# atunnd/Hair-centric-Image-Retrieval

Hardware: AMD Instinct MI355X
Metric: query-images/sec (embed+top-10) ViT-B/16 vs 1M gallery, 1/2/4/8 GPU (higher is better)
Workload: dtype f16; 1 GPU; ViT-B/16 (HSimCLR ViTWrapper, random init) embed + top-10 over 1000000 x 768 f32 gallery row-sharded over 1 GPU(s); query_batch_per_gpu=880, global_query_batch=880, gallery_rows=1000000, gallery_dtype=f32, topk=10, sim_mode=filtered, residual_stream=f16, steps_in_flight=2, parallelism=gallery-shard1+query-dp1

## Files before the change

### hair-centric-image-retrieval_amd/csrc/gemm.hip

```cpp
#include "sim_core.h"
#include "act.h"
#include "gemm_plan.h"
#include <stdlib.h>

namespace {

using GemmCfg = SimCfg<_Float16, 2, 2, 2>;

constexpr int EPI_RESID_F16_STATS = 7;
constexpr int EPI_LN_BIAS_F16 = 8;
constexpr int EPI_LN_BIAS_GELU_F16 = 9;
constexpr int EPI_BIAS_F16_DUAL_GELU = 10;

struct GemmArgs {
  const _Float16* a;
  const _Float16* w;
  const float* bias;
  const float* scale;
  void* out;
  int64_t m, lda, ldw, ldo;
  int n, k;
  const float* ln_stats;
  const float* ln_c1;
  float* stats_part;
  const void* resid;
  void* out2;
  int64_t stats_ld = 0;
};

__device__ __forceinline__ int xcd_remap(int bid, int nwg) {
  const int q = nwg >> 3, r = nwg & 7, xcd = bid & 7, j = bid >> 3;
  return (xcd < r ? xcd * (q + 1) : r * (q + 1) + (xcd - r) * q) + j;
}

template <int EPI, int NTILES>
// ... 70 lines not shown
  gemm_epilogue_t<EPI, 2>(g, acc, m0, n0 + wave_n * 64, wave_m, lane);
}
__device__ __forceinline__ void launder(f32x4& v) { asm volatile("" : "+v"(v)); }

struct WaveAcc {
  f32x4 a[8][4];
  __device__ __forceinline__ void zero() {
#pragma unroll
    for (int x = 0; x < 8; ++x)
#pragma unroll
      for (int y = 0; y < 4; ++y)
#pragma unroll
        for (int i = 0; i < 4; ++i) a[x][y][i] = 0.f;
  }
};

__device__ __forceinline__ float sum8_dpp(float v) {
  v += __builtin_bit_cast(float, __builtin_amdgcn_update_dpp(0, __builtin_bit_cast(int, v), 0xB1, 0xF, 0xF, true));
  v += __builtin_bit_cast(float, __builtin_amdgcn_update_dpp(0, __builtin_bit_cast(int, v), 0x4E, 0xF, 0xF, true));
  v += __builtin_bit_cast(float, __builtin_amdgcn_update_dpp(0, __builtin_bit_cast(int, v), 0x141, 0xF, 0xF, true));
  return v;
}


template <int EPI, bool FULL, int NTW, int MTT, int MTH>
__device__ __forceinline__ void gemm_epilogue_lds_impl(const GemmArgs& g, const f32x4 (&acc)[NTW][MTT], int mt0,
                                                       char* region, int64_t m0w, int nbase, int lane) {
  constexpr bool kLn = (EPI == EPI_LN_BIAS_F16 || EPI == EPI_LN_BIAS_GELU_F16);
  constexpr bool kGelu = (EPI == HCIR_EPI_BIAS_GELU_F16 || EPI == EPI_LN_BIAS_GELU_F16);
  constexpr bool kResidH = (EPI == HCIR_EPI_BIAS_RESID_F16 || EPI == EPI_RESID_F16_STATS);
  constexpr bool kDual = (EPI == EPI_BIAS_F16_DUAL_GELU);
  constexpr bool kF16 = (EPI == HCIR_EPI_BIAS_F16 || kGelu || kLn ||
                         EPI == HCIR_EPI_AFFINE_RELU_F16 || kResidH || kDual);
  constexpr bool kAffine = (EPI == HCIR_EPI_AFFINE_RELU_F16 || EPI == HCIR_EPI_AFFINE_F32);
  constexpr int FPP = kF16 ? 64 : 32;
  constexpr int NPASS = NTW * 16 / FPP;
  constexpr int NIT = MTH * 2;
  constexpr int UB = (NIT % 4 == 0) ? 4 : 3;
  static_assert(NIT % UB == 0 && (NTW * 16) % FPP == 0, "geometry");
  const int rrow = lane >> 3, rchunk = lane & 7;

  constexpr bool kScaleA = kF16 && (EPI == HCIR_EPI_AFFINE_RELU_F16 || kResidH);
  f32x4 biasA[kF16 ? NTW : 1], scaleA[kScaleA ? NTW : 1];
  bool has_scale = false;
  if constexpr (kF16) {
    has_scale = kScaleA && (EPI == HCIR_EPI_AFFINE_RELU_F16 || g.scale != nullptr);
#pragma unroll
    for (int t = 0; t < NTW; ++t) {
      const int n = nbase + 16 * t + 4 * (lane >> 4);
      biasA[t] = (f32x4){0.f, 0.f, 0.f, 0.f};
      if (g.bias) biasA[t] = *reinterpret_cast<const f32x4*>(g.bias + n);
      if constexpr (kScaleA) {
        scaleA[t] = (f32x4){1.f, 1.f, 1.f, 1.f};
        if (has_scale) scaleA[t] = *reinterpret_cast<const f32x4*>(g.scale + n);
      }
    }
// ... 6 lines not shown
#pragma unroll
    for (int j = 0; j < NB; ++j) {
      const int n = nbase + pass * FPP + rchunk * (kF16 ? 8 : 4) + 4 * j;
      bias[pass][j] = (f32x4){0.f, 0.f, 0.f, 0.f};
      scale[pass][j] = (f32x4){1.f, 1.f, 1.f, 1.f};
      if (g.bias) bias[pass][j] = *reinterpret_cast<const f32x4*>(g.bias + n);
      if (kAffine || (EPI == HCIR_EPI_BIAS_RESID_F32 && g.scale))
        scale[pass][j] = *reinterpret_cast<const f32x4*>(g.scale + n);
    }
  }
  float ln_rs[MTH], ln_mean[MTH];
  f32x4 c1a[NTW];
  if constexpr (kLn) {
#pragma unroll
    for (int mt = 0; mt < MTH; ++mt) {
      int64_t mm = m0w + 16 * mt + (lane & 15);
      mm = mm < g.m ? mm : g.m - 1;
      ln_mean[mt] = g.ln_stats[2 * mm];
      ln_rs[mt] = g.ln_stats[2 * mm + 1];
    }
#pragma unroll
    for (int t = 0; t < NTW; ++t) c1a[t] = *reinterpret_cast<const f32x4*>(g.ln_c1 + nbase + 16 * t + 4 * (lane >> 4));
  }
  asm volatile("s_waitcnt vmcnt(0)" ::: "memory");
  if constexpr (kLn) {
#pragma unroll
    for (int mt = 0; mt < MTH; ++mt) asm volatile("" : "+v"(ln_rs[mt]));
#pragma unroll
    for (int mt = 0; mt < MTH; ++mt) asm volatile("" : "+v"(ln_mean[mt]));
#pragma unroll
    for (int t = 0; t < NTW; ++t) launder(c1a[t]);
  }
  if constexpr (kF16) {
#pragma unroll
    for (int t = 0; t < NTW; ++t) {
      launder(biasA[t]);
      if constexpr (kScaleA) launder(scaleA[t]);
    }
  } else {
#pragma unroll
    for (int pass = 0; pass < NPASS; ++pass)
#pragma unroll
      for (int j = 0; j < NB; ++j) {
        launder(bias[pass][j]);
        launder(scale[pass][j]);
      }
  }

  constexpr int NITER = kDual ? 2 * NPASS : NPASS;
#pragma unroll
  for (int iter = 0; iter < NITER; ++iter) {
    const int pass = kDual ? iter >> 1 : iter;
    const bool second = kDual && (iter & 1);
    const int r16 = lane & 15, q16 = lane >> 4;
#pragma unroll
    for (int mt = 0; mt < MTH; ++mt) {
      const int row = mt * 16 + r16;
      if constexpr (kF16) {
#pragma unroll
        for (int q = 0; q < 4; ++q) {
          const int nt = 4 * pass + q;
          f16x4 o;
          float xs[4];
#pragma unroll
          for (int e = 0; e < 4; ++e) {
            float x = acc[nt][mt0 + mt][e];
            const float bb = biasA[nt][e];
            if constexpr (kLn) {
              x = __builtin_fmaf(ln_rs[mt], __builtin_fmaf(-ln_mean[mt], c1a[nt][e], x), bb);
            } else if constexpr (EPI == HCIR_EPI_AFFINE_RELU_F16) {
              x = fmaxf(__builtin_fmaf(x, scaleA[nt][e], bb), 0.f);
            } else if constexpr (kResidH) {
              x = scaleA[nt][e] * (x + bb);
            } else {
              x += bb;
            }
            xs[e] = x;
          }
          if (kGelu || second) {
#pragma unroll
            for (int e = 0; e < 4; e += 2) {
              const gelu_f32x2 y = gelu_erf2((gelu_f32x2){xs[e], xs[e + 1]});
              xs[e] = y[0];
              xs[e + 1] = y[1];
            }
          }
#pragma unroll
          for (int e = 0; e < 4; ++e) o[e] = (_Float16)xs[e];
          const int chunk = 2 * q + (q16 >> 1);
          *reinterpret_cast<f16x4*>(region + row * 128 + ((chunk ^ (row & 7)) << 4) + 8 * (q16 & 1)) = o;
        }
      } else {
#pragma unroll
        for (int q = 0; q < 2; ++q) {
          const int nt = 2 * pass + q;
          const int chunk = 4 * q + q16;
// ... 5 lines not shown
      const int n = nbase + pass * 64 + rchunk * 8;
#pragma unroll
      for (int it0 = 0; it0 < NIT; it0 += UB) {
        f16x8 oldh[UB];
        if constexpr (kResidH) {
#pragma unroll
          for (int u = 0; u < UB; ++u) {
            const int64_t mm = m0w + (it0 + u) * 8 + rrow;
#pragma unroll
            for (int e = 0; e < 8; ++e) oldh[u][e] = (_Float16)0.f;
            if (FULL || mm < g.m)
              oldh[u] = *reinterpret_cast<const f16x8*>(static_cast<const _Float16*>(g.resid) + mm * g.ldo + n);
          }
        }
#pragma unroll
        for (int u = 0; u < UB; ++u) {
          const int row = (it0 + u) * 8 + rrow;
          const f16x8 v = *reinterpret_cast<const f16x8*>(region + row * 128 + ((rchunk ^ (row & 7)) << 4));
          f16x8 o;
          if constexpr (kResidH)
            o = v + oldh[u];
          else
            o = v;
          const int64_t m = m0w + row;
          if (FULL || m < g.m)
            __builtin_nontemporal_store(
                o, reinterpret_cast<f16x8*>(static_cast<_Float16*>(second ? g.out2 : g.out) + m * g.ldo + n));
          if constexpr (EPI == EPI_RESID_F16_STATS) {
            float xv[8], s1 = 0.f;
#pragma unroll
            for (int e = 0; e < 8; ++e) {
              xv[e] = (float)o[e];
              s1 += xv[e];
            }
            const float mean_s = sum8_dpp(s1) * (1.0f / 64.0f);
            float m2 = 0.f;
#pragma unroll
            for (int e = 0; e < 8; ++e) {
              const float dv = xv[e] - mean_s;
              m2 = __builtin_fmaf(dv, dv, m2);
            }
            m2 = sum8_dpp(m2);
            if (rchunk == 0 && (FULL || m < g.m)) {
              const int64_t slice = (nbase >> 6) + pass;
              *reinterpret_cast<f32x2*>(g.stats_part + (slice * (g.stats_ld ? g.stats_ld : g.m) + m) * 2) = (f32x2){mean_s, m2};
            }
          }
        }
      }
    } else {
      const int n = nbase + pass * 32 + rchunk * 4;
      const f32x4 b = bias[pass][0], sc = scale[pass][0];
#pragma unroll
      for (int it0 = 0; it0 < NIT; it0 += UB) {
        f32x4 oldv[UB];
#pragma unroll
        for (int u = 0; u < UB; ++u) {
          const int64_t mm = m0w + (it0 + u) * 8 + rrow;
          oldv[u] = (f32x4){0.f, 0.f, 0.f, 0.f};
          if constexpr (EPI == HCIR_EPI_BIAS_RESID_F32) {
            if (FULL || mm < g.m)
              oldv[u] = *reinterpret_cast<const f32x4*>(static_cast<const float*>(g.resid) + mm * g.ldo + n);
          }
        }
#pragma unroll
        for (int u = 0; u < UB; ++u) {
          const int row = (it0 + u) * 8 + rrow;
          const int64_t mm = m0w + row;
          f32x4 v = *reinterpret_cast<const f32x4*>(region + row * 128 + ((rchunk ^ (row & 7)) << 4));
          if constexpr (EPI == HCIR_EPI_AFFINE_F32) {
#pragma unroll
            for (int e = 0; e < 4; ++e) v[e] = __builtin_fmaf(v[e], sc[e], b[e]);
          } else if constexpr (EPI == HCIR_EPI_BIAS_RESID_F32) {
#pragma unroll
            for (int e = 0; e < 4; ++e) v[e] = __builtin_fmaf(sc[e], v[e] + b[e], oldv[u][e]);
          } else {
#pragma unroll
            for (int e = 0; e < 4; ++e) v[e] += b[e];
          }
          if (FULL || mm < g.m) *reinterpret_cast<f32x4*>(static_cast<float*>(g.out) + mm * g.ldo + n) = v;
        }
      }
    }
  }
}

template <int EPI, int NTW, int MTT, int MTH>
__device__ __forceinline__ void gemm_epilogue_lds(const GemmArgs& g, const f32x4 (&acc)[NTW][MTT], int mt0,
                                                  char* region, int64_t m0w, int nbase, int lane) {
  asm volatile("" : "+v"(lane));
  if (m0w + 16 * MTH <= g.m)
    gemm_epilogue_lds_impl<EPI, true, NTW, MTT, MTH>(g, acc, mt0, region, m0w, nbase, lane);
  else
    gemm_epilogue_lds_impl<EPI, false, NTW, MTT, MTH>(g, acc, mt0, region, m0w, nbase, lane);
}

template <int EPI, bool GLDS>
__global__ __launch_bounds__(256, 2) void gemm_f16_kernel(GemmArgs g, int tiles_n, int tiles_m) {
  using Cfg = GemmCfg;
  __shared__ __attribute__((aligned(16))) char lds[Cfg::LDS_BYTES];
  const int tid = threadIdx.x, lane = tid & 63, wave = tid >> 6;
  const int wave_n = wave >> 1, wave_m = wave & 1;
  const int t = xcd_remap(blockIdx.x, tiles_n * tiles_m);
  const int tn = t % tiles_n, tm = t / tiles_n;
  const int n0 = tn * 128;
  const int64_t m0 = (int64_t)tm * 128;
  const int nkc = (g.k + 63) / 64;

  f32x16 acc[2][2];
#pragma unroll
  for (int a = 0; a < 2; ++a)
// ... 447 lines not shown
#pragma unroll
        for (int e = 0; e < 4; ++e) v[e] = acc[nt][mt][4 * grp + e] + b[e] + p.pos_mult * ps[e];
        if constexpr (sizeof(TokT) == 4) {
          *reinterpret_cast<f32x4*>(orow + n) = v;
        } else {
          f16x4 o;
#pragma unroll
          for (int e = 0; e < 4; ++e) o[e] = (_Float16)v[e];
          *reinterpret_cast<f16x4*>(orow + n) = o;
        }
      }
    }
  }
}

template <typename TokT>
__global__ void cls_row_kernel(const float* __restrict__ cls, const float* __restrict__ pos,
                               float pos_mult, int64_t b, int t, int d, TokT* __restrict__ tok) {
  const int64_t i = (int64_t)blockIdx.x * blockDim.x + threadIdx.x;
  if (i >= b * d) return;
  const int64_t bi = i / d;
  const int n = (int)(i % d);
  tok[bi * t * (int64_t)d + n] = (TokT)(cls[n] + pos_mult * pos[n]);
}

__global__ void ln_stats_finalize_kernel(const float* __restrict__ part, int parts, int64_t m, float slice_n,
                                         float eps, float* __restrict__ stats) {
  const int64_t row = (int64_t)blockIdx.x * blockDim.x + threadIdx.x;
  if (row >= m) return;
  float ms = 0.f;
  for (int p = 0; p < parts; ++p) ms += part[((int64_t)p * m + row) * 2];
  const float mean = ms / (float)parts;
  float m2 = 0.f;
  for (int p = 0; p < parts; ++p) {
    const f32x2 v = *reinterpret_cast<const f32x2*>(part + ((int64_t)p * m + row) * 2);
    const float dm = v[0] - mean;
    m2 += v[1] + slice_n * dm * dm;
  }
  const float var = m2 / (slice_n * (float)parts);
  *reinterpret_cast<f32x2*>(stats + 2 * row) = (f32x2){mean, 1.0f / sqrtf(var + eps)};
}

template <int EPI>
void launch_gemm_mid(const GemmArgs& g, hipStream_t st) {
  const int tn = g.n / GMid::TN, tm = (int)hcir_cdiv(g.m, GMid::TM);
  const int grid = tn * tm < 512 ? tn * tm : 512;
// ... 124 lines not shown

int hcir_gemm_f16_fused(const void* a, int64_t lda, const void* w, int64_t ldw, const float* bias,
                        const float* scale, int64_t m, int32_t n, int32_t k, int epilogue, void* out,
                        int64_t ldo, const float* ln_stats, const float* ln_c1, float* stats_part,
                        void* stream) {
  HCIR_ENTER();
  if (!a || !w || !out || m <= 0 || n <= 0 || k <= 0) return HCIR_ERR_INVALID;
  if ((k & 7) || (n & 7) || lda < k || ldw < k || (lda & 7) || (ldw & 7) || ldo < n || (ldo & 7))
    return HCIR_ERR_INVALID;
  const bool ln = ln_stats || ln_c1;
  if (ln && (!ln_stats || !ln_c1 || !bias)) return HCIR_ERR_INVALID;
  if (ln && stats_part) return HCIR_ERR_INVALID;
  if (!ln && !stats_part) return HCIR_ERR_INVALID;
  if (ln && epilogue != HCIR_EPI_BIAS_F16 && epilogue != HCIR_EPI_BIAS_GELU_F16) return HCIR_ERR_UNSUPPORTED;
  if (stats_part && epilogue != HCIR_EPI_BIAS_RESID_F16) return HCIR_ERR_UNSUPPORTED;
  if (!gemm_takes_big(m, n, k)) return HCIR_ERR_UNSUPPORTED;
  GemmArgs g{static_cast<const _Float16*>(a), static_cast<const _Float16*>(w), bias, scale, out, m,
             lda, ldw, ldo, n, k, ln_stats, ln_c1, stats_part, out, nullptr};
  hipStream_t st = static_cast<hipStream_t>(stream);
  const GemmPlan p = gemm_plan(m, n, k, false);
  if (stats_part) launch_gemm_big<EPI_RESID_F16_STATS>(g, p, st);
  else if (epilogue == HCIR_EPI_BIAS_F16) launch_gemm_big<EPI_LN_BIAS_F16>(g, p, st);
  else launch_gemm_big<EPI_LN_BIAS_GELU_F16>(g, p, st);
  HCIR_LAUNCH_CHECK();
  return HCIR_OK;
}

int hcir_ln_stats_finalize(const float* stats_part, int32_t slices, int64_t m, int32_t n_features, float eps,
                           float* ln_stats, void* stream) {
  HCIR_ENTER();
  if (!stats_part || !ln_stats || slices <= 0 || m <= 0 || n_features <= 0) return HCIR_ERR_INVALID;
  if ((int64_t)slices * 64 != n_features) return HCIR_ERR_INVALID;
  hipLaunchKernelGGL(ln_stats_finalize_kernel, dim3((unsigned)hcir_cdiv(m, 256)), dim3(256), 0,
                     static_cast<hipStream_t>(stream), stats_part, slices, m, 64.0f, eps, ln_stats);
  HCIR_LAUNCH_CHECK();
  return HCIR_OK;
}

int hcir_patch_embed(const float* img, int64_t b, int32_t c, int32_t h, int32_t w_px, int32_t p,
                     const void* w_f16, int64_t ldw, const float* bias, const float* cls,
                     const float* pos, float pos_mult, int32_t d, void* tok, int tok_dtype,
                     void* stream) {
  HCIR_ENTER();
  if (!img || !w_f16 || !bias || !cls || !pos || !tok || b <= 0) return HCIR_ERR_INVALID;
  if (p <= 0 || p > 32 || c <= 0 || h % p || w_px % p || (d & 7)) return HCIR_ERR_INVALID;
  const int kreal = c * p * p;
// ... 6 lines not shown
  if (tok_dtype != HCIR_F32 && tok_dtype != HCIR_F16) return HCIR_ERR_UNSUPPORTED;
  const dim3 cgrid((unsigned)hcir_cdiv(b * d, 256));
  if (tok_dtype == HCIR_F32) {
    if (p == 16)
      hipLaunchKernelGGL((patch_embed_kernel<float, true>), dim3(tiles_n * tiles_m), dim3(256), 0, st, a, tiles_n, tiles_m);
    else
      hipLaunchKernelGGL((patch_embed_kernel<float, false>), dim3(tiles_n * tiles_m), dim3(256), 0, st, a, tiles_n, tiles_m);
    HCIR_LAUNCH_CHECK();
    hipLaunchKernelGGL(cls_row_kernel<float>, cgrid, dim3(256), 0, st, cls, pos, pos_mult, b, np + 1, d,
                       static_cast<float*>(tok));
  } else {
    if (p == 16)
      hipLaunchKernelGGL((patch_embed_kernel<_Float16, true>), dim3(tiles_n * tiles_m), dim3(256), 0, st, a, tiles_n, tiles_m);
    else
      hipLaunchKernelGGL((patch_embed_kernel<_Float16, false>), dim3(tiles_n * tiles_m), dim3(256), 0, st, a, tiles_n, tiles_m);
    HCIR_LAUNCH_CHECK();
    hipLaunchKernelGGL(cls_row_kernel<_Float16>, cgrid, dim3(256), 0, st, cls, pos, pos_mult, b, np + 1, d,
                       static_cast<_Float16*>(tok));
  }
  HCIR_LAUNCH_CHECK();
  return HCIR_OK;
}

}
```

### hair-centric-image-retrieval_amd/hcir/_lib.py

```python
from __future__ import annotations

import ctypes
import os
import subprocess

import torch

_PKG_DIR = os.path.dirname(os.path.dirname(os.path.abspath(__file__)))
CSRC_DIR = os.path.join(_PKG_DIR, "csrc")
LIB_PATH = os.environ.get("HCIR_LIB_PATH") or os.path.join(CSRC_DIR, "libhcir.so")

F32, F16, BF16 = 0, 1, 2
EPI_BIAS_F16, EPI_BIAS_GELU_F16, EPI_BIAS_RESID_F32, EPI_BIAS_F32, EPI_AFFINE_RELU_F16, EPI_AFFINE_F32, \
    EPI_BIAS_RESID_F16 = range(7)
GEMM_ROUTE_SMALL, GEMM_ROUTE_MID, GEMM_ROUTE_BIG, GEMM_ROUTE_SPLIT = range(4)
GEMM_ROUTE_EPI_DUAL = 10

_lib = None

c_i32, c_i64, c_f32, c_vp, c_sz, c_int = (
    ctypes.c_int32, ctypes.c_int64, ctypes.c_float, ctypes.c_void_p, ctypes.c_size_t, ctypes.c_int)
c_f64 = ctypes.c_double

SIGNATURES = {
    "hcir_version": (c_int, []),
    "hcir_status_string": (ctypes.c_char_p, [c_int]),
    "hcir_build_id": (ctypes.c_char_p, []),
    "hcir_row_invnorm": (c_int, [c_vp, c_i64, c_i32, c_i64, c_int, c_f32, c_vp, c_vp]),
    "hcir_l2_normalize": (c_int, [c_vp, c_i64, c_i32, c_f32, c_vp, c_vp, c_vp]),
    "hcir_sim_topk_workspace_bytes": (c_sz, [c_i64, c_i64, c_i32, c_i32, c_int]),
    "hcir_sim_topk": (c_int, [c_vp, c_i64, c_vp, c_i64, c_i32, c_i32, c_int, c_vp, c_vp, c_i64,
                              c_vp, c_vp, c_vp, c_sz, c_vp]),
    "hcir_topk_refine_f32": (c_int, [c_vp, c_i64, c_vp, c_i64, c_i32, c_vp, c_vp, c_i32, c_i32, c_i64, c_vp, c_vp,
                                     c_vp, c_vp, c_vp, c_vp, c_vp, c_vp]),
    "hcir_topk_merge": (c_int, [c_vp, c_vp, c_i32, c_i64, c_i32, c_i32, c_vp, c_vp, c_vp]),
    "hcir_ntxent_workspace_bytes": (c_sz, [c_i64, c_i32, c_int]),
    "hcir_ntxent_fwd": (c_int, [c_vp, c_vp, c_i64, c_i32, c_int, c_f32, c_vp, c_vp, c_vp, c_sz, c_vp]),
    "hcir_ntxent_bwd_workspace_bytes": (c_sz, [c_i64, c_i32, c_int]),
    "hcir_ntxent_bwd": (c_int, [c_vp, c_vp, c_i64, c_i32, c_int, c_f32, c_vp, c_f32, c_vp, c_vp, c_vp, c_sz, c_vp]),
    "hcir_layernorm_f16": (c_int, [c_vp, c_int, c_i64, c_i32, c_i64, c_vp, c_vp, c_f32, c_vp, c_i64, c_vp]),
    "hcir_gemm_f16": (c_int, [c_vp, c_i64, c_vp, c_i64, c_vp, c_vp, c_i64, c_i32, c_i32, c_int,
                              c_vp, c_i64, c_vp]),
    "hcir_gemm_f16_resid": (c_int, [c_vp, c_i64, c_vp, c_i64, c_vp, c_vp, c_i64, c_i32, c_i32, c_int, c_vp,
                                    c_vp, c_i64, c_vp]),
    "hcir_gemm_f16_gelu_dual": (c_int, [c_vp, c_i64, c_vp, c_i64, c_vp, c_i64, c_i32, c_i32, c_vp, c_vp, c_i64, c_vp]),
    "hcir_gemm_fused_supported": (c_int, [c_i64, c_i32, c_i32]),
    "hcir_gemm_stats_slices": (c_i32, [c_i32]),
    "hcir_gemm_route": (c_int, [c_i64, c_i32, c_i32, c_int, c_vp]),
    "hcir_gemm_f16_fused": (c_int, [c_vp, c_i64, c_vp, c_i64, c_vp, c_vp, c_i64, c_i32, c_i32, c_int,
                                    c_vp, c_i64, c_vp, c_vp, c_vp, c_vp]),
    "hcir_ln_stats_finalize": (c_int, [c_vp, c_i32, c_i64, c_i32, c_f32, c_vp, c_vp]),
    "hcir_patch_embed": (c_int, [c_vp, c_i64, c_i32, c_i32, c_i32, c_i32, c_vp, c_i64, c_vp, c_vp, c_vp,
                                 c_f32, c_i32, c_vp, c_int, c_vp]),
    "hcir_attn_fwd": (c_int, [c_vp, c_i64, c_i32, c_i32, c_i32, c_f32, c_i32, c_vp, c_vp]),
    "hcir_cls_head": (c_int, [c_vp, c_int, c_i64, c_i32, c_i32, c_vp, c_vp, c_f32, c_int, c_vp, c_vp, c_vp]),
    "hcir_patch_mean": (c_int, [c_vp, c_int, c_i64, c_i32, c_i32, c_vp, c_vp, c_f32, c_vp, c_vp]),
    "hcir_knn_transform_u8": (c_int, [c_vp, c_i64, c_i32, c_i32, c_i32, c_vp, c_vp, c_vp, c_vp]),
    "hcir_ema_update": (c_int, [c_vp, c_vp, c_vp, c_i64, c_f32, c_f32, c_vp]),
    "hcir_grad_sumsq": (c_int, [c_vp, c_vp, c_i64, c_vp, c_vp, c_vp, c_vp]),
    "hcir_optim_finalize": (c_int, [c_vp, c_vp, c_i64, c_vp, c_vp, c_f32, c_f32, c_i32, c_int, c_f64, c_vp, c_vp,
                                    c_i32, c_f64, c_f64, c_vp, c_i32, c_vp, c_vp, c_vp, c_vp, c_vp]),
    "hcir_adam_step": (c_int, [c_vp, c_vp, c_vp, c_vp, c_vp, c_vp, c_vp, c_i64, c_vp, c_vp, c_vp, c_f32, c_f32,
                               c_f32, c_f32, c_vp]),
    "hcir_positive_masking": (c_int, [c_vp, c_i64, c_i32, c_i32, c_i32, c_i32, c_f32, c_vp, c_vp, c_vp, c_vp,
                                      c_vp]),
    "hcir_convert_f32": (c_int, [c_vp, c_i64, c_int, c_vp, c_vp]),
    "hcir_gelu_fwd_f16": (c_int, [c_vp, c_i64, c_vp, c_vp]),
    "hcir_gelu_bwd_f16": (c_int, [c_vp, c_vp, c_i64, c_vp, c_vp]),
    "hcir_add_f32_f16": (c_int, [c_vp, c_vp, c_i64, c_vp, c_vp]),
    "hcir_layernorm_bwd_blocks": (c_i32, [c_i64]),
    "hcir_layernorm_bwd": (c_int, [c_vp, c_int, c_i64, c_i32, c_i64, c_vp, c_i64, c_vp, c_f32, c_vp, c_vp, c_i64,
                                   c_vp, c_vp, c_int, c_vp, c_sz, c_vp]),
    "hcir_layernorm_bwd_fused": (c_int, [c_vp, c_int, c_i64, c_i32, c_i64, c_vp, c_i64, c_vp, c_f32, c_vp, c_vp,
                                         c_i64, c_vp, c_vp, c_int, c_vp, c_i64, c_vp, c_vp, c_sz, c_vp]),
    "hcir_gelu_bwd_colsum_f16": (c_int, [c_vp, c_vp, c_i64, c_i32, c_i64, c_vp, c_vp, c_int, c_vp, c_sz, c_vp]),
    "hcir_colsum_chunks": (c_i32, [c_i64]),
# ... 116 lines not shown
```

### hair-centric-image-retrieval_amd/hcir/vit_engine.py

```python
from __future__ import annotations

from dataclasses import dataclass, field
from typing import List, Optional

import torch

from . import _lib
from ._lib import HcirError, check
from .ops import _ptr


import os as _os

DEFAULT_RESID_DTYPE = torch.float16 if _os.environ.get("HCIR_RESID", "f32") == "f16" else torch.float32
LN_FUSE = _os.environ.get("HCIR_LN_FUSE", "1") != "0"


@dataclass
class VitLayer:
    ln1_w: torch.Tensor
    ln1_b: torch.Tensor
    qkv_w: torch.Tensor
    qkv_b: Optional[torch.Tensor]
    proj_w: torch.Tensor
# ... 94 lines not shown
        self._bufs = {}
        self.prof = None

    def _mark(self, name: str) -> None:
        if self.prof is not None:
            self.prof.mark(name)

    def _buffers(self, b: int, t: int, slot: int = 0):
        key = (b, t, slot)
        bufs = self._bufs.get(key)
        if bufs is None:
            m, d, dev = b * t, self.dim, self.device
            bufs = dict(
                tok=torch.empty((b, t, d), dtype=self.resid_dtype, device=dev),
                ln=torch.empty((m, d), dtype=torch.float16, device=dev),
                qkv=torch.empty((m, 3 * d), dtype=torch.float16, device=dev),
                att=torch.empty((m, d), dtype=torch.float16, device=dev),
                hid=torch.empty((m, self.mlp), dtype=torch.float16, device=dev),
                att_c=torch.empty((b, d), dtype=torch.float16, device=dev),
                ln_c=torch.empty((b, d), dtype=torch.float16, device=dev),
                hid_c=torch.empty((b, self.mlp), dtype=torch.float16, device=dev),
                stats_part=torch.empty((max(d // 64, 1), m, 2), dtype=torch.float32, device=dev),
                stats=torch.empty((m, 2), dtype=torch.float32, device=dev),
            )
            self._bufs = {k: v for k, v in self._bufs.items() if k[2] != slot}
            self._bufs[key] = bufs
        return bufs

    def forward_tokens(self, x: torch.Tensor, cls_only_last: bool = False, slot: int = 0) -> torch.Tensor:
        if not x.is_cuda:
            raise HcirError(f"input is on {x.device}; the hcir ViT runs on a HIP device only")
        if x.dtype != torch.float32:
            x = x.float()
        x = x.contiguous()
        b, c, hh, ww = x.shape
        ps = self.patch
        if hh % ps or ww % ps:
            raise HcirError("image sides must be multiples of the patch size")
        t = (hh // ps) * (ww // ps) + 1
        if t > 288:
            raise HcirError("hcir_attn_fwd supports up to 288 tokens")
        if t != self.pos.shape[0]:
            raise HcirError(f"image gives {t} tokens but pos_embedding has {self.pos.shape[0]}")
        L, d, m = self.L, self.dim, b * t
        st = torch.cuda.current_stream(x.device).cuda_stream
        w = self._buffers(b, t, slot)
        tok, ln, qkv, att, hid = w["tok"], w["ln"], w["qkv"], w["att"], w["hid"]
        check(L.hcir_patch_embed(x.data_ptr(), b, c, hh, ww, ps, self.conv_w.data_ptr(), self.conv_w.shape[1],
                                 self.conv_b.data_ptr(), self.cls.data_ptr(), self.pos.data_ptr(),
                                 self.pos_mult, d, tok.data_ptr(), self._rt, st), "hcir_patch_embed")
        self._mark("patch_embed")
        scale = (d // self.heads) ** -0.5
        last = len(self.layers) - 1
        fuse = (LN_FUSE and self.resid_dtype == torch.float16
                and L.hcir_gemm_fused_supported(m, 3 * d, d) and L.hcir_gemm_fused_supported(m, d, d)
                and L.hcir_gemm_fused_supported(m, self.mlp, d) and L.hcir_gemm_fused_supported(m, d, self.mlp))
        sp, stats = w["stats_part"], w["stats"]
        nsl = d // 64
        have_stats = False

        def resid_gemm(a, k, wt, bias, ls, rows, pitch, want_stats, what):
            if want_stats:
                check(L.hcir_gemm_f16_fused(a.data_ptr(), k, wt.data_ptr(), k, bias.data_ptr(), _ptr(ls), m, d, k,
                                            _lib.EPI_BIAS_RESID_F16, tok.data_ptr(), d, None, None, sp.data_ptr(),
                                            st), what)
                check(L.hcir_ln_stats_finalize(sp.data_ptr(), nsl, m, d, self.eps, stats.data_ptr(), st),
                      "hcir_ln_stats_finalize")
            else:
                check(L.hcir_gemm_f16(a.data_ptr(), k, wt.data_ptr(), k, bias.data_ptr(), _ptr(ls), rows, d, k,
                                      self._resid_epi, tok.data_ptr(), pitch, st), what)

        for li, l in enumerate(self.layers):
            if fuse and have_stats:
                check(L.hcir_gemm_f16_fused(tok.data_ptr(), d, l.qkv_wg.data_ptr(), d, l.qkv_c2.data_ptr(), None,
                                            m, 3 * d, d, _lib.EPI_BIAS_F16, qkv.data_ptr(), 3 * d,
                                            stats.data_ptr(), l.qkv_c1.data_ptr(), None, st),
                      "hcir_gemm_f16_fused(ln1+qkv)")
            else:
                check(L.hcir_layernorm_f16(tok.data_ptr(), self._rt, m, d, d, l.ln1_w.data_ptr(),
                                           l.ln1_b.data_ptr(), self.eps, ln.data_ptr(), d, st), "hcir_layernorm_f16")
                self._mark("layernorm")
                check(L.hcir_gemm_f16(ln.data_ptr(), d, l.qkv_w.data_ptr(), d, _ptr(l.qkv_b), None, m, 3 * d, d,
                                      _lib.EPI_BIAS_F16, qkv.data_ptr(), 3 * d, st), "hcir_gemm_f16(qkv)")
            self._mark("gemm_qkv")
            if cls_only_last and li == last:
                rows, pitch, nq, att_r, ln_r, hid_r, fz = b, t * d, 1, w["att_c"], w["ln_c"], w["hid_c"], False
            else:
                rows, pitch, nq, att_r, ln_r, hid_r, fz = m, d, t, att, ln, hid, fuse
            check(L.hcir_attn_fwd(qkv.data_ptr(), b, t, self.heads, d // self.heads, scale, nq, att_r.data_ptr(), st),
                  "hcir_attn_fwd")
            self._mark("attn")
            resid_gemm(att_r, d, l.proj_w, l.proj_b, l.ls1, rows, pitch, fz, "hcir_gemm_f16(proj)")
            self._mark("gemm_proj")
            if fz:
                check(L.hcir_gemm_f16_fused(tok.data_ptr(), d, l.fc1_wg.data_ptr(), d, l.fc1_c2.data_ptr(), None,
                                            m, self.mlp, d, _lib.EPI_BIAS_GELU_F16, hid.data_ptr(), self.mlp,
                                            stats.data_ptr(), l.fc1_c1.data_ptr(), None, st),
                      "hcir_gemm_f16_fused(ln2+fc1)")
            else:
                check(L.hcir_layernorm_f16(tok.data_ptr(), self._rt, rows, d, pitch, l.ln2_w.data_ptr(),
                                           l.ln2_b.data_ptr(), self.eps, ln_r.data_ptr(), d, st), "hcir_layernorm_f16")
                self._mark("layernorm")
                check(L.hcir_gemm_f16(ln_r.data_ptr(), d, l.fc1_w.data_ptr(), d, l.fc1_b.data_ptr(), None, rows,
                                      self.mlp, d, _lib.EPI_BIAS_GELU_F16, hid_r.data_ptr(), self.mlp, st),
                      "hcir_gemm_f16(fc1)")
            self._mark("gemm_fc1")
# ... 46 lines not shown
```

### include/hcir.h

```cpp
#ifndef HCIR_H
#define HCIR_H

#include <stddef.h>
#include <stdint.h>

#ifdef __cplusplus
extern "C" {
#endif

typedef enum {
  HCIR_OK = 0,
  HCIR_ERR_INVALID = -1,
  HCIR_ERR_UNSUPPORTED = -2,
  HCIR_ERR_LAUNCH = -3,
  HCIR_ERR_WORKSPACE = -4
} hcir_status;

typedef enum {
  HCIR_F32 = 0,
  HCIR_F16 = 1,
  HCIR_BF16 = 2
} hcir_dtype;

int hcir_version(void);
// ... 54 lines not shown
                  const float* bias, const float* scale, int64_t m, int32_t n,
                  int32_t k, int epilogue, void* out, int64_t ldo, void* stream);
int hcir_gemm_f16_resid(const void* a, int64_t lda, const void* w, int64_t ldw, const float* bias,
                        const float* scale, int64_t m, int32_t n, int32_t k, int epilogue, const void* resid,
                        void* out, int64_t ldo, void* stream);

int hcir_gemm_f16_gelu_dual(const void* a, int64_t lda, const void* w, int64_t ldw, const float* bias, int64_t m,
                            int32_t n, int32_t k, void* out_pre, void* out_act, int64_t ldo, void* stream);

int hcir_gemm_fused_supported(int64_t m, int32_t n, int32_t k);
int32_t hcir_gemm_stats_slices(int32_t n);
typedef enum {
  HCIR_GEMM_ROUTE_SMALL = 0,
  HCIR_GEMM_ROUTE_MID = 1,
  HCIR_GEMM_ROUTE_BIG = 2,
  HCIR_GEMM_ROUTE_SPLIT = 3
} hcir_gemm_route_kind;
#define HCIR_GEMM_ROUTE_EPI_DUAL 10
int hcir_gemm_route(int64_t m, int32_t n, int32_t k, int epilogue, int64_t* rows_on_big);
int hcir_gemm_f16_fused(const void* a, int64_t lda, const void* w, int64_t ldw, const float* bias,
                        const float* scale, int64_t m, int32_t n, int32_t k, int epilogue,
                        void* out, int64_t ldo, const float* ln_stats, const float* ln_c1,
                        float* stats_part, void* stream);
int hcir_ln_stats_finalize(const float* stats_part, int32_t slices, int64_t m, int32_t n_features,
                           float eps, float* ln_stats, void* stream);

int hcir_patch_embed(const float* img, int64_t b, int32_t c, int32_t h, int32_t w_px,
                     int32_t p, const void* w_f16, int64_t ldw, const float* bias,
                     const float* cls, const float* pos, float pos_mult, int32_t d, void* tok,
                     int tok_dtype, void* stream);

int hcir_attn_fwd(const void* qkv, int64_t b, int32_t t, int32_t h, int32_t hd,
                  float scale, int32_t nq, void* out, void* stream);

int hcir_cls_head(const void* tok, int tok_dtype, int64_t b, int32_t t, int32_t d,
                  const float* gamma, const float* beta, float eps, int l2_normalize,
                  float* emb_f32, void* emb_f16, void* stream);

int hcir_patch_mean(const void* tok, int tok_dtype, int64_t b, int32_t t, int32_t d,
                    const float* gamma, const float* beta, float eps, float* out_f32,
                    void* stream);

int hcir_knn_transform_u8(const uint8_t* img, int64_t b, int32_t h, int32_t w, int32_t size,
                          const float* mean3, const float* std3, float* out, void* stream);

int hcir_ema_update(const uint64_t* dst_ptrs, const uint64_t* src_ptrs, const int64_t* counts,
                    int64_t n_chunks, float m, float one_minus_m, void* stream);


int hcir_grad_sumsq(const uint64_t* g_ptrs, const int64_t* counts, int64_t n_chunks, const float* scale,
                    float* partial, int32_t* flags, void* stream);

int hcir_optim_finalize(const float* partial, const int32_t* flags, int64_t n_chunks, float* scale,
// ... 274 lines not shown
```

Measured before the change: 25860 query-images/sec.

## Fuse patch embedding into big GEMM with im2col gather; trim last-layer QKV to class rows

Adds a 256x256-tile patch-embed GEMM kernel that gathers image pixels directly from f32 input into LDS (implicit im2col), applies bias plus position embedding in the epilogue, and scatters rows past the class token slot. A separate small kernel writes the class rows. In the last layer, when only the class token is needed, the fused LN+QKV GEMM computes K/V columns for all rows but Q only for class rows, via a new mid-tile LN GEMM entry point. This removes the separate patch-embed path and the unused Q work at the cost of more complex gather indexing and an extra launch.

After: 26170 query-images/sec (median of 6 runs). 1.01x the previous value.

```diff
diff --git a/hair-centric-image-retrieval_amd/csrc/gemm.hip b/hair-centric-image-retrieval_amd/csrc/gemm.hip
--- a/hair-centric-image-retrieval_amd/csrc/gemm.hip
+++ b/hair-centric-image-retrieval_amd/csrc/gemm.hip
@@ -1,6 +1,7 @@
 #include "sim_core.h"
 #include "act.h"
 #include "gemm_plan.h"
+#include "patch_plan.h"
 #include <stdlib.h>
 
 namespace {
@@ -11,6 +12,7 @@
 constexpr int EPI_LN_BIAS_F16 = 8;
 constexpr int EPI_LN_BIAS_GELU_F16 = 9;
 constexpr int EPI_BIAS_F16_DUAL_GELU = 10;
+constexpr int EPI_PATCH_F16_STATS = 11;
 
 struct GemmArgs {
   const _Float16* a;
@@ -127,16 +129,53 @@
   return v;
 }
 
-
-template <int EPI, bool FULL, int NTW, int MTT, int MTH>
-__device__ __forceinline__ void gemm_epilogue_lds_impl(const GemmArgs& g, const f32x4 (&acc)[NTW][MTT], int mt0,
+__device__ __forceinline__ f32x2 slice_stats8(const f16x8& o) {
+  float xv[8], s1 = 0.f;
+#pragma unroll
+  for (int e = 0; e < 8; ++e) {
+    xv[e] = (float)o[e];
+    s1 += xv[e];
+  }
+  const float mean_s = sum8_dpp(s1) * (1.0f / 64.0f);
+  float m2 = 0.f;
+#pragma unroll
+  for (int e = 0; e < 8; ++e) {
+    const float dv = xv[e] - mean_s;
+    m2 = __builtin_fmaf(dv, dv, m2);
+  }
+  return (f32x2){mean_s, sum8_dpp(m2)};
+}
+
+struct PatchRowMap {
+  int mb, bi0, rem0, np;
+  float inv;
+  __device__ __forceinline__ PatchRowMap() : mb(0), bi0(0), rem0(0), np(1), inv(1.f) {}
+  __device__ __forceinline__ PatchRowMap(int64_t m0w, int64_t mtot, int np_) : np(np_) {
+    mb = (int)(m0w < mtot ? m0w : mtot - 1);
+    bi0 = mb / np;
+    rem0 = mb - bi0 * np;
+    inv = 1.0f / (float)np;
+  }
+  __device__ __forceinline__ void map(int64_t m, int64_t mtot, int& bi, int& pi) const {
+    const int r = rem0 + ((int)(m < mtot ? m : mtot - 1) - mb);
+    int q = (int)((float)r * inv);
+    q += ((q + 1) * np <= r) ? 1 : 0;
+    q -= (q * np > r) ? 1 : 0;
+    bi = bi0 + q;
+    pi = r - q * np;
+  }
+};
+
+template <int EPI, bool FULL, int NTW, int MTT, int MTH, class GA>
+__device__ __forceinline__ void gemm_epilogue_lds_impl(const GA& g, const f32x4 (&acc)[NTW][MTT], int mt0,
                                                        char* region, int64_t m0w, int nbase, int lane) {
   constexpr bool kLn = (EPI == EPI_LN_BIAS_F16 || EPI == EPI_LN_BIAS_GELU_F16);
   constexpr bool kGelu = (EPI == HCIR_EPI_BIAS_GELU_F16 || EPI == EPI_LN_BIAS_GELU_F16);
   constexpr bool kResidH = (EPI == HCIR_EPI_BIAS_RESID_F16 || EPI == EPI_RESID_F16_STATS);
   constexpr bool kDual = (EPI == EPI_BIAS_F16_DUAL_GELU);
+  constexpr bool kPatch = (EPI == EPI_PATCH_F16_STATS);
   constexpr bool kF16 = (EPI == HCIR_EPI_BIAS_F16 || kGelu || kLn ||
-                         EPI == HCIR_EPI_AFFINE_RELU_F16 || kResidH || kDual);
+                         EPI == HCIR_EPI_AFFINE_RELU_F16 || kResidH || kDual || kPatch);
   constexpr bool kAffine = (EPI == HCIR_EPI_AFFINE_RELU_F16 || EPI == HCIR_EPI_AFFINE_F32);
   constexpr int FPP = kF16 ? 64 : 32;
   constexpr int NPASS = NTW * 16 / FPP;
@@ -189,6 +228,8 @@
 #pragma unroll
     for (int t = 0; t < NTW; ++t) c1a[t] = *reinterpret_cast<const f32x4*>(g.ln_c1 + nbase + 16 * t + 4 * (lane >> 4));
   }
+  PatchRowMap rm;
+  if constexpr (kPatch) rm = PatchRowMap(m0w, g.m, g.np);
   asm volatile("s_waitcnt vmcnt(0)" ::: "memory");
   if constexpr (kLn) {
 #pragma unroll
@@ -224,6 +265,14 @@
     for (int mt = 0; mt < MTH; ++mt) {
       const int row = mt * 16 + r16;
       if constexpr (kF16) {
+        f32x4 posA[kPatch ? 4 : 1];
+        if constexpr (kPatch) {
+          int bi, pi;
+          rm.map(m0w + row, g.m, bi, pi);
+          const float* prow = g.pos + (int64_t)(1 + pi) * g.n + nbase + 64 * pass + 4 * q16;
+#pragma unroll
+          for (int q = 0; q < 4; ++q) posA[q] = *reinterpret_cast<const f32x4*>(prow + 16 * q);
+        }
 #pragma unroll
         for (int q = 0; q < 4; ++q) {
           const int nt = 4 * pass + q;
@@ -239,6 +288,8 @@
               x = fmaxf(__builtin_fmaf(x, scaleA[nt][e], bb), 0.f);
             } else if constexpr (kResidH) {
               x = scaleA[nt][e] * (x + bb);
+            } else if constexpr (kPatch) {
+              x = __builtin_fmaf(g.pos_mult, posA[q][e], x + bb);
             } else {
               x += bb;
             }
@@ -290,28 +341,21 @@
             o = v + oldh[u];
           else
             o = v;
-          const int64_t m = m0w + row;
-          if (FULL || m < g.m)
+          int64_t m = m0w + row;
+          const int64_t mrow = m;
+          if constexpr (kPatch) {
+            int bi, pi;
+            rm.map(m, g.m, bi, pi);
+            m = (int64_t)bi * (g.np + 1) + 1 + pi;
+          }
+          if (FULL || mrow < g.m)
             __builtin_nontemporal_store(
                 o, reinterpret_cast<f16x8*>(static_cast<_Float16*>(second ? g.out2 : g.out) + m * g.ldo + n));
-          if constexpr (EPI == EPI_RESID_F16_STATS) {
-            float xv[8], s1 = 0.f;
-#pragma unroll
-            for (int e = 0; e < 8; ++e) {
-              xv[e] = (float)o[e];
-              s1 += xv[e];
-            }
-            const float mean_s = sum8_dpp(s1) * (1.0f / 64.0f);
-            float m2 = 0.f;
-#pragma unroll
-            for (int e = 0; e < 8; ++e) {
-              const float dv = xv[e] - mean_s;
-              m2 = __builtin_fmaf(dv, dv, m2);
-            }
-            m2 = sum8_dpp(m2);
-            if (rchunk == 0 && (FULL || m < g.m)) {
+          if constexpr (EPI == EPI_RESID_F16_STATS || kPatch) {
+            const f32x2 ss = slice_stats8(o);
+            if (rchunk == 0 && (FULL || mrow < g.m) && (!kPatch || g.stats_part)) {
               const int64_t slice = (nbase >> 6) + pass;
-              *reinterpret_cast<f32x2*>(g.stats_part + (slice * (g.stats_ld ? g.stats_ld : g.m) + m) * 2) = (f32x2){mean_s, m2};
+              *reinterpret_cast<f32x2*>(g.stats_part + (slice * (g.stats_ld ? g.stats_ld : g.m) + m) * 2) = ss;
             }
           }
         }
@@ -353,8 +397,8 @@
   }
 }
 
-template <int EPI, int NTW, int MTT, int MTH>
-__device__ __forceinline__ void gemm_epilogue_lds(const GemmArgs& g, const f32x4 (&acc)[NTW][MTT], int mt0,
+template <int EPI, int NTW, int MTT, int MTH, class GA>
+__device__ __forceinline__ void gemm_epilogue_lds(const GA& g, const f32x4 (&acc)[NTW][MTT], int mt0,
                                                   char* region, int64_t m0w, int nbase, int lane) {
   asm volatile("" : "+v"(lane));
   if (m0w + 16 * MTH <= g.m)
@@ -848,6 +892,166 @@
   const int64_t bi = i / d;
   const int n = (int)(i % d);
   tok[bi * t * (int64_t)d + n] = (TokT)(cls[n] + pos_mult * pos[n]);
+}
+
+struct PatchGemmArgs : GemmArgs {
+  const float* img;
+  const float* pos;
+  float pos_mult;
+  int np, gw, c, h, w_px;
+};
+
+__global__ __launch_bounds__(512, 2) void patch_embed_big_kernel(PatchGemmArgs g, int tiles_n, int tiles_m) {
+  __shared__ __attribute__((aligned(16))) char lds[2 * G256::STAGE_BYTES];
+
+  const int tid = threadIdx.x, lane = tid & 63, wave = tid >> 6;
+  const int wave_n = wave / G256::WAVES_M, wave_m = wave % G256::WAVES_M;
+  GemmStages<G256> stg(g, lds, tiles_n, tiles_m, tid);
+  const int nkc = stg.nkc, nsteps = stg.nsteps;
+  constexpr int NA = G256::NLOAD - G256::NW;
+
+  const char* ibase = nullptr;
+  uint32_t aoff[NA];
+  auto set_rows = [&](int t_i) {
+    int n0;
+    int64_t m0;
+    stg.tile_origin(t_i, n0, m0);
+    int otid = tid;
+    asm volatile("" : "+v"(otid));
+    const int chunk = otid & 7;
+    const int bfirst = (int)m0 / g.np;
+    ibase = reinterpret_cast<const char*>(g.img + (int64_t)bfirst * g.c * g.h * g.w_px);
+#pragma unroll
+    for (int i = 0; i < NA; ++i) {
+      int64_t m = m0 + (otid >> 3) + 64 * i;
+      m = m < g.m ? m : g.m - 1;
+      const int mi = (int)m;
+      const int bi = mi / g.np, pi = mi - bi * g.np;
+      const int py = pi / g.gw, px = pi - py * g.gw;
+      aoff[i] = (uint32_t)((((bi - bfirst) * g.c * g.h + py * 16 + (chunk >> 1)) * g.w_px + px * 16 + 8 * (chunk & 1)) * 4);
+    }
+  };
+  f32x4 stage_a[2 * NA];
+  auto gather_load = [&](int kc) {
+    const char* kbase = ibase + ((int64_t)(kc >> 2) * g.h + 4 * (kc & 3)) * g.w_px * 4;
+#pragma unroll
+    for (int i = 0; i < NA; ++i) {
+      stage_a[2 * i] = *reinterpret_cast<const f32x4*>(kbase + aoff[i]);
+      stage_a[2 * i + 1] = *reinterpret_cast<const f32x4*>(kbase + aoff[i] + 16);
+    }
+  };
+  auto gather_store = [&](int slot) {
+#pragma unroll
+    for (int i = 0; i < NA; ++i) {
+      f16x8 v;
+#pragma unroll
+      for (int e = 0; e < 4; ++e) {
+        v[e] = (_Float16)stage_a[2 * i][e];
+        v[4 + e] = (_Float16)stage_a[2 * i + 1][e];
+      }
+      *reinterpret_cast<f16x8*>(lds + slot * G256::STAGE_BYTES + sim_slot_off(G256::TN + (tid >> 3) + 64 * i, tid & 7)) = v;
+    }
+  };
+
+  WaveAcc acc;
+  acc.zero();
+
+  if (nsteps > 0) {
+    stg.set_sources(0);
+    set_rows(0);
+    gather_load(0);
+#pragma unroll
+    for (int i = 0; i < G256::NW; ++i) stg.issue_piece(0, i);
+    gather_store(0);
+    stg.issue_advance();
+    if (stg.issue_kc == 0 && stg.issue_ti < stg.my_tiles) set_rows(stg.issue_ti);
+  }
+
+  int kc = 0, ti = 0;
+  for (int step = 0; step < nsteps; ++step) {
+    asm volatile("s_waitcnt vmcnt(0) lgkmcnt(0)" ::: "memory");
+    __builtin_amdgcn_s_barrier();
+
+    const char* st = lds + (step & 1) * G256::STAGE_BYTES;
+    const bool do_issue = step + 1 < nsteps;
+    const int islot = (step + 1) & 1;
+    const int r16 = lane & 15, kq = lane >> 4;
+    if (do_issue) gather_load(stg.issue_kc);
+#pragma unroll
+    for (int ks2 = 0; ks2 < 2; ++ks2) {
+      const int chunk = 4 * ks2 + kq;
+      u32x4 bf[4];
+#pragma unroll
+      for (int mt = 0; mt < 4; ++mt)
+        bf[mt] = *reinterpret_cast<const u32x4*>(st + sim_slot_off(G256::TN + wave_m * 64 + mt * 16 + r16, chunk));
+#pragma unroll
+      for (int half = 0; half < 2; ++half) {
+        u32x4 af[4];
+#pragma unroll
+        for (int q = 0; q < 4; ++q)
+          af[q] = *reinterpret_cast<const u32x4*>(
+              st + sim_slot_off(wave_n * 128 + (4 * half + q) * 16 + r16, chunk));
+        if (do_issue && ks2 == 0 && half == 0) {
+#pragma unroll
+          for (int i = 0; i < G256::NW; ++i) stg.issue_piece(islot, i);
+        }
+#pragma unroll
+        for (int q = 0; q < 4; ++q)
+#pragma unroll
+          for (int mt = 0; mt < 4; ++mt)
+            acc.a[4 * half + q][mt] = __builtin_amdgcn_mfma_f32_16x16x32_f16(
+                __builtin_bit_cast(f16x8, af[q]), __builtin_bit_cast(f16x8, bf[mt]), acc.a[4 * half + q][mt],
+                0, 0, 0);
+      }
+    }
+    if (do_issue) {
+      gather_store(islot);
+      stg.issue_advance();
+      if (stg.issue_kc == 0 && stg.issue_ti < stg.my_tiles) set_rows(stg.issue_ti);
+    }
+
+    if (++kc == nkc) {
+      int n0;
+      int64_t m0;
+      stg.tile_origin(ti, n0, m0);
+      __builtin_amdgcn_s_barrier();
+      gemm_epilogue_lds<EPI_PATCH_F16_STATS, 8, 4, 4>(g, acc.a, 0, lds + (step & 1) * G256::STAGE_BYTES + wave * 8192,
+                                                      m0 + wave_m * 64, n0 + wave_n * 128, lane);
+      acc.zero();
+      kc = 0;
+      ++ti;
+      if (stg.issue_ti < stg.my_tiles) {
+        stg.set_sources(stg.issue_ti);
+        set_rows(stg.issue_ti);
+      }
+    }
+  }
+}
+
+__global__ __launch_bounds__(256) void cls_row_stats_kernel(const float* __restrict__ cls, const float* __restrict__ pos,
+                                                            float pos_mult, int64_t b, int t, int d,
+                                                            _Float16* __restrict__ tok, float* __restrict__ stats_part) {
+  const int per = d >> 3;
+  const int64_t total = b * per;
+  int64_t i = (int64_t)blockIdx.x * blockDim.x + threadIdx.x;
+  const bool inside = i < total;
+  i = inside ? i : total - 1;
+  const int64_t bi = i / per;
+  const int n = (int)(i - bi * per) * 8;
+  f16x8 o;
+#pragma unroll
+  for (int j = 0; j < 2; ++j) {
+    const f32x4 cv = *reinterpret_cast<const f32x4*>(cls + n + 4 * j);
+    const f32x4 pv = *reinterpret_cast<const f32x4*>(pos + n + 4 * j);
+#pragma unroll
+    for (int e = 0; e < 4; ++e) o[4 * j + e] = (_Float16)__builtin_fmaf(pos_mult, pv[e], cv[e]);
+  }
+  const f32x2 ss = slice_stats8(o);
+  if (!inside) return;
+  const int64_t row = bi * t;
+  *reinterpret_cast<f16x8*>(tok + row * d + n) = o;
+  if (stats_part && (threadIdx.x & 7) == 0)
+    *reinterpret_cast<f32x2*>(stats_part + ((int64_t)(n >> 6) * (b * t) + row) * 2) = ss;
 }
 
 __global__ void ln_stats_finalize_kernel(const float* __restrict__ part, int parts, int64_t m, float slice_n,
@@ -1018,6 +1222,21 @@
   if (stats_part) launch_gemm_big<EPI_RESID_F16_STATS>(g, p, st);
   else if (epilogue == HCIR_EPI_BIAS_F16) launch_gemm_big<EPI_LN_BIAS_F16>(g, p, st);
   else launch_gemm_big<EPI_LN_BIAS_GELU_F16>(g, p, st);
+  HCIR_LAUNCH_CHECK();
+  return HCIR_OK;
+}
+
+int hcir_gemm_f16_ln_rows(const void* a, int64_t lda, const void* w, int64_t ldw, const float* bias, int64_t m,
+                          int32_t n, int32_t k, void* out, int64_t ldo, const float* ln_stats, const float* ln_c1,
+                          void* stream) {
+  HCIR_ENTER();
+  if (!a || !w || !out || !bias || !ln_stats || !ln_c1 || m <= 0 || n <= 0 || k <= 0) return HCIR_ERR_INVALID;
+  if (lda < k || ldw < k || (lda & 7) || (ldw & 7) || ldo < n || (ldo & 7)) return HCIR_ERR_INVALID;
+  if (k % 64 || n % GMid::TN) return HCIR_ERR_UNSUPPORTED;
+  if ((n / GMid::TN) * hcir_cdiv(m, GMid::TM) > 0x7fffffff) return HCIR_ERR_INVALID;
+  GemmArgs g{static_cast<const _Float16*>(a), static_cast<const _Float16*>(w), bias, nullptr, out, m,
+             lda, ldw, ldo, n, k, ln_stats, ln_c1, nullptr, out, nullptr};
+  launch_gemm_mid<EPI_LN_BIAS_F16>(g, static_cast<hipStream_t>(stream));
   HCIR_LAUNCH_CHECK();
   return HCIR_OK;
 }
@@ -1070,4 +1289,52 @@
   return HCIR_OK;
 }
 
-}
+int hcir_patch_embed_route(int64_t b, int32_t c, int32_t h, int32_t w_px, int32_t p, int32_t d, int64_t ldw,
+                           int tok_dtype) {
+  if (b <= 0 || c <= 0 || h <= 0 || w_px <= 0 || p <= 0 || d <= 0 || h % p || w_px % p) return HCIR_ERR_INVALID;
+  return patch_embed_plan(b, c, h, w_px, p, d, ldw, tok_dtype).route;
+}
+
+int hcir_patch_embed_fused(const float* img, int64_t b, int32_t c, int32_t h, int32_t w_px, int32_t p,
+                           const void* w_f16, int64_t ldw, const float* bias, const float* cls, const float* pos,
+                           float pos_mult, int32_t d, void* tok, int tok_dtype, float* stats_part, void* stream) {
+  HCIR_ENTER();
+  if (!img || !w_f16 || !bias || !cls || !pos || !tok || b <= 0) return HCIR_ERR_INVALID;
+  if (p <= 0 || p > 32 || c <= 0 || h <= 0 || w_px <= 0 || h % p || w_px % p || d <= 0 || (d & 7))
+    return HCIR_ERR_INVALID;
+  if (tok_dtype != HCIR_F32 && tok_dtype != HCIR_F16) return HCIR_ERR_UNSUPPORTED;
+  const PatchPlan q = patch_embed_plan(b, c, h, w_px, p, d, ldw, tok_dtype);
+  if (q.route != HCIR_PATCH_ROUTE_BIG) return HCIR_ERR_UNSUPPORTED;
+  PatchGemmArgs g{};
+  g.a = nullptr;
+  g.w = static_cast<const _Float16*>(w_f16);
+  g.bias = bias;
+  g.scale = nullptr;
+  g.out = tok;
+  g.m = q.rows;
+  g.lda = 0;
+  g.ldw = ldw;
+  g.ldo = d;
+  g.n = d;
+  g.k = c * 256;
+  g.stats_part = stats_part;
+  g.resid = tok;
+  g.stats_ld = b * q.t;
+  g.img = img;
+  g.pos = pos;
+  g.pos_mult = pos_mult;
+  g.np = q.np;
+  g.gw = w_px / 16;
+  g.c = c;
+  g.h = h;
+  g.w_px = w_px;
+  hipStream_t st = static_cast<hipStream_t>(stream);
+  hipLaunchKernelGGL(patch_embed_big_kernel, dim3(q.grid), dim3(G256::NT), 0, st, g, q.tn, q.tm);
+  HCIR_LAUNCH_CHECK();
+  hipLaunchKernelGGL(cls_row_stats_kernel, dim3((unsigned)hcir_cdiv(b * (d >> 3), 256)), dim3(256), 0, st, cls, pos,
+                     pos_mult, b, q.t, d, static_cast<_Float16*>(tok), stats_part);
+  HCIR_LAUNCH_CHECK();
+  return HCIR_OK;
+}
+
+}
diff --git a/hair-centric-image-retrieval_amd/csrc/patch_plan.h b/hair-centric-image-retrieval_amd/csrc/patch_plan.h
--- /dev/null
+++ b/hair-centric-image-retrieval_amd/csrc/patch_plan.h
@@ -0,0 +1,40 @@
+#pragma once
+#include <stdint.h>
+
+#include "../../include/hcir.h"
+
+constexpr int PATCH_BIG_TN = 256, PATCH_BIG_TM = 256;
+constexpr int PATCH_BIG_GRID = 256;
+
+struct PatchPlan {
+  int route;
+  int np, t;
+  int64_t rows;
+  int tn, tm;
+  int grid;
+};
+
+static inline int64_t patch_token_row(int64_t m, int np) { return m + m / np + 1; }
+
+static inline PatchPlan patch_embed_plan(int64_t b, int c, int h, int w_px, int p, int d, int64_t ldw, int tok_dtype) {
+  PatchPlan q;
+  q.route = HCIR_PATCH_ROUTE_TILE128;
+  q.np = 0;
+  q.t = 0;
+  q.rows = 0;
+  q.tn = q.tm = q.grid = 0;
+  if (b <= 0 || c <= 0 || p <= 0 || h <= 0 || w_px <= 0 || d <= 0 || h % p || w_px % p) return q;
+  q.np = (h / p) * (w_px / p);
+  q.t = q.np + 1;
+  q.rows = b * q.np;
+  if (p != 16 || tok_dtype != HCIR_F16 || d % PATCH_BIG_TN || ldw != (int64_t)c * 256) return q;
+  if (b * q.t > 0x7fffffff - PATCH_BIG_TM) return q;
+  if ((int64_t)c * (256 + 2 * (int64_t)q.np) * 1024 > 0x7fffffff) return q;
+  const int64_t tiles = (int64_t)(d / PATCH_BIG_TN) * ((q.rows + PATCH_BIG_TM - 1) / PATCH_BIG_TM);
+  if (tiles > 0x7fffffff) return q;
+  q.route = HCIR_PATCH_ROUTE_BIG;
+  q.tn = d / PATCH_BIG_TN;
+  q.tm = (int)((q.rows + PATCH_BIG_TM - 1) / PATCH_BIG_TM);
+  q.grid = tiles < PATCH_BIG_GRID ? (int)tiles : PATCH_BIG_GRID;
+  return q;
+}
diff --git a/hair-centric-image-retrieval_amd/hcir/_lib.py b/hair-centric-image-retrieval_amd/hcir/_lib.py
--- a/hair-centric-image-retrieval_amd/hcir/_lib.py
+++ b/hair-centric-image-retrieval_amd/hcir/_lib.py
@@ -15,6 +15,8 @@
     EPI_BIAS_RESID_F16 = range(7)
 GEMM_ROUTE_SMALL, GEMM_ROUTE_MID, GEMM_ROUTE_BIG, GEMM_ROUTE_SPLIT = range(4)
 GEMM_ROUTE_EPI_DUAL = 10
+PATCH_ROUTE_TILE128, PATCH_ROUTE_BIG = range(2)
+ERR_UNSUPPORTED = -2
 
 _lib = None
 
@@ -49,9 +51,13 @@
     "hcir_gemm_route": (c_int, [c_i64, c_i32, c_i32, c_int, c_vp]),
     "hcir_gemm_f16_fused": (c_int, [c_vp, c_i64, c_vp, c_i64, c_vp, c_vp, c_i64, c_i32, c_i32, c_int,
                                     c_vp, c_i64, c_vp, c_vp, c_vp, c_vp]),
+    "hcir_gemm_f16_ln_rows": (c_int, [c_vp, c_i64, c_vp, c_i64, c_vp, c_i64, c_i32, c_i32, c_vp, c_i64, c_vp, c_vp, c_vp]),
     "hcir_ln_stats_finalize": (c_int, [c_vp, c_i32, c_i64, c_i32, c_f32, c_vp, c_vp]),
     "hcir_patch_embed": (c_int, [c_vp, c_i64, c_i32, c_i32, c_i32, c_i32, c_vp, c_i64, c_vp, c_vp, c_vp,
                                  c_f32, c_i32, c_vp, c_int, c_vp]),
+    "hcir_patch_embed_route": (c_int, [c_i64, c_i32, c_i32, c_i32, c_i32, c_i32, c_i64, c_int]),
+    "hcir_patch_embed_fused": (c_int, [c_vp, c_i64, c_i32, c_i32, c_i32, c_i32, c_vp, c_i64, c_vp, c_vp, c_vp,
+                                       c_f32, c_i32, c_vp, c_int, c_vp, c_vp]),
     "hcir_attn_fwd": (c_int, [c_vp, c_i64, c_i32, c_i32, c_i32, c_f32, c_i32, c_vp, c_vp]),
     "hcir_cls_head": (c_int, [c_vp, c_int, c_i64, c_i32, c_i32, c_vp, c_vp, c_f32, c_int, c_vp, c_vp, c_vp]),
     "hcir_patch_mean": (c_int, [c_vp, c_int, c_i64, c_i32, c_i32, c_vp, c_vp, c_f32, c_vp, c_vp]),
diff --git a/hair-centric-image-retrieval_amd/hcir/vit_engine.py b/hair-centric-image-retrieval_amd/hcir/vit_engine.py
--- a/hair-centric-image-retrieval_amd/hcir/vit_engine.py
+++ b/hair-centric-image-retrieval_amd/hcir/vit_engine.py
@@ -140,6 +140,7 @@
                 hid_c=torch.empty((b, self.mlp), dtype=torch.float16, device=dev),
                 stats_part=torch.empty((max(d // 64, 1), m, 2), dtype=torch.float32, device=dev),
                 stats=torch.empty((m, 2), dtype=torch.float32, device=dev),
+                stats_c=torch.empty((b, 2), dtype=torch.float32, device=dev),
             )
             self._bufs = {k: v for k, v in self._bufs.items() if k[2] != slot}
             self._bufs[key] = bufs
@@ -164,10 +165,6 @@
         st = torch.cuda.current_stream(x.device).cuda_stream
         w = self._buffers(b, t, slot)
         tok, ln, qkv, att, hid = w["tok"], w["ln"], w["qkv"], w["att"], w["hid"]
-        check(L.hcir_patch_embed(x.data_ptr(), b, c, hh, ww, ps, self.conv_w.data_ptr(), self.conv_w.shape[1],
-                                 self.conv_b.data_ptr(), self.cls.data_ptr(), self.pos.data_ptr(),
-                                 self.pos_mult, d, tok.data_ptr(), self._rt, st), "hcir_patch_embed")
-        self._mark("patch_embed")
         scale = (d // self.heads) ** -0.5
         last = len(self.layers) - 1
         fuse = (LN_FUSE and self.resid_dtype == torch.float16
@@ -176,6 +173,18 @@
         sp, stats = w["stats_part"], w["stats"]
         nsl = d // 64
         have_stats = False
+        kpad = self.conv_w.shape[1]
+        if fuse and L.hcir_patch_embed_route(b, c, hh, ww, ps, d, kpad, self._rt) == _lib.PATCH_ROUTE_BIG:
+            check(L.hcir_patch_embed_fused(x.data_ptr(), b, c, hh, ww, ps, self.conv_w.data_ptr(), kpad,
+                                           self.conv_b.data_ptr(), self.cls.data_ptr(), self.pos.data_ptr(),
+                                           self.pos_mult, d, tok.data_ptr(), self._rt, None, st),
+                  "hcir_patch_embed_fused")
+            self._mark("patch_embed")
+        else:
+            check(L.hcir_patch_embed(x.data_ptr(), b, c, hh, ww, ps, self.conv_w.data_ptr(), kpad,
+                                     self.conv_b.data_ptr(), self.cls.data_ptr(), self.pos.data_ptr(),
+                                     self.pos_mult, d, tok.data_ptr(), self._rt, st), "hcir_patch_embed")
+            self._mark("patch_embed")
 
         def resid_gemm(a, k, wt, bias, ls, rows, pitch, want_stats, what):
             if want_stats:
@@ -188,11 +197,16 @@
                 check(L.hcir_gemm_f16(a.data_ptr(), k, wt.data_ptr(), k, bias.data_ptr(), _ptr(ls), rows, d, k,
                                       self._resid_epi, tok.data_ptr(), pitch, st), what)
 
+        def off(tensor, elems):
+            return None if tensor is None else tensor.data_ptr() + elems * tensor.element_size()
+
         for li, l in enumerate(self.layers):
+            cls_last = cls_only_last and li == last and fuse and have_stats
+            c0 = d if cls_last else 0
             if fuse and have_stats:
-                check(L.hcir_gemm_f16_fused(tok.data_ptr(), d, l.qkv_wg.data_ptr(), d, l.qkv_c2.data_ptr(), None,
-                                            m, 3 * d, d, _lib.EPI_BIAS_F16, qkv.data_ptr(), 3 * d,
-                                            stats.data_ptr(), l.qkv_c1.data_ptr(), None, st),
+                check(L.hcir_gemm_f16_fused(tok.data_ptr(), d, off(l.qkv_wg, c0 * d), d, off(l.qkv_c2, c0), None,
+                                            m, 3 * d - c0, d, _lib.EPI_BIAS_F16, off(qkv, c0), 3 * d,
+                                            stats.data_ptr(), off(l.qkv_c1, c0), None, st),
                       "hcir_gemm_f16_fused(ln1+qkv)")
             else:
                 check(L.hcir_layernorm_f16(tok.data_ptr(), self._rt, m, d, d, l.ln1_w.data_ptr(),
@@ -200,6 +214,11 @@
                 self._mark("layernorm")
                 check(L.hcir_gemm_f16(ln.data_ptr(), d, l.qkv_w.data_ptr(), d, _ptr(l.qkv_b), None, m, 3 * d, d,
                                       _lib.EPI_BIAS_F16, qkv.data_ptr(), 3 * d, st), "hcir_gemm_f16(qkv)")
+            if cls_last:
+                w["stats_c"].copy_(stats.view(b, t, 2)[:, 0])
+                check(L.hcir_gemm_f16_ln_rows(tok.data_ptr(), t * d, l.qkv_wg.data_ptr(), d, l.qkv_c2.data_ptr(), b, d,
+                                              d, qkv.data_ptr(), t * 3 * d, w["stats_c"].data_ptr(),
+                                              l.qkv_c1.data_ptr(), st), "hcir_gemm_f16_ln_rows(q, class rows)")
             self._mark("gemm_qkv")
             if cls_only_last and li == last:
                 rows, pitch, nq, att_r, ln_r, hid_r, fz = b, t * d, 1, w["att_c"], w["ln_c"], w["hid_c"], False
diff --git a/include/hcir.h b/include/hcir.h
--- a/include/hcir.h
+++ b/include/hcir.h
@@ -100,6 +100,9 @@
                         const float* scale, int64_t m, int32_t n, int32_t k, int epilogue,
                         void* out, int64_t ldo, const float* ln_stats, const float* ln_c1,
                         float* stats_part, void* stream);
+int hcir_gemm_f16_ln_rows(const void* a, int64_t lda, const void* w, int64_t ldw, const float* bias, int64_t m,
+                          int32_t n, int32_t k, void* out, int64_t ldo, const float* ln_stats,
+                          const float* ln_c1, void* stream);
 int hcir_ln_stats_finalize(const float* stats_part, int32_t slices, int64_t m, int32_t n_features,
                            float eps, float* ln_stats, void* stream);
 
@@ -107,6 +110,16 @@
                      int32_t p, const void* w_f16, int64_t ldw, const float* bias,
                      const float* cls, const float* pos, float pos_mult, int32_t d, void* tok,
                      int tok_dtype, void* stream);
+typedef enum {
+  HCIR_PATCH_ROUTE_TILE128 = 0,
+  HCIR_PATCH_ROUTE_BIG = 1
+} hcir_patch_route_kind;
+int hcir_patch_embed_route(int64_t b, int32_t c, int32_t h, int32_t w_px, int32_t p, int32_t d, int64_t ldw,
+                           int tok_dtype);
+int hcir_patch_embed_fused(const float* img, int64_t b, int32_t c, int32_t h, int32_t w_px,
+                           int32_t p, const void* w_f16, int64_t ldw, const float* bias,
+                           const float* cls, const float* pos, float pos_mult, int32_t d, void* tok,
+                           int tok_dtype, float* stats_part, void* stream);
 
 int hcir_attn_fwd(const void* qkv, int64_t b, int32_t t, int32_t h, int32_t hd,
                   float scale, int32_t nq, void* out, void* stream);
```
